# pylat/adaptive-proximal-algorithms

Hardware: NVIDIA B200
Metric: AdaPGM iters/sec on 65536x131072 fp64 lasso (higher is better)
Workload: dtype f64

## Files before the change

adaptive-proximal-algorithms_b200/csrc/api.cu:

```cuda
#include <algorithm>
#include <cmath>
#include <cstdlib>
#include <cstring>
#include <numeric>
#include "context.hpp"
#include "ops.cuh"
#include "solver_pd.cuh"
#include "solver_pg.cuh"
#include "solver_mp.cuh"
#include "solver_fused.cuh"
#include "solver_resident.cuh"
#include "solver_gridres.cuh"
#include "comm.hpp"

using namespace adaprox;

static int64_t round_up(int64_t v, int64_t a) { return (v + a - 1) / a * a; }

static int ws_reset(adaprox_ctx* h, size_t need) {
  if (need > h->ws_bytes) {
    if (h->ws) cudaFree(h->ws);
    h->ws = nullptr; h->ws_bytes = 0;
    size_t want = need + (need >> 3) + (1u << 20);
    cudaError_t e = cudaMalloc(&h->ws, want);
// ... 578 lines not shown
  if (cooperative && !std::getenv("ADAPROX_FUSED_NONCOOP")) {
    attrs[1].id = cudaLaunchAttributeCooperative;
    attrs[1].val.cooperative = 1;
    cfg->numAttrs = 2;
  }
  return ADAPROX_OK;
}

struct FusedPlan {
  cudaLaunchConfig_t cfg;
  cudaLaunchAttribute attrs[2];
  int Q = 0;
  int G = 0;
  FusedArgs fa{};
};
static int fused_plan(adaprox_ctx* h, const void* kernel, const DProblem& P, bool cooperative, FusedPlan* pl) {
  pl->fa = FusedArgs{};
  pl->fa.C = fused_cluster_size(P);
  int rc = fused_config(h, kernel, pl->fa.C, cooperative, &pl->cfg, pl->attrs, &pl->Q);
  if (rc) return rc;
  pl->G = pl->fa.C * pl->Q;
  pl->fa.tagged = cooperative ? 1 : 0;
  pl->fa.hV = 0; pl->fa.hR = 16;
#if ADAPROX_FUSED_VARIANT == 1
  if (cooperative && pl->fa.C == kFMaxCluster) {
    int V = (h->sm_count - pl->G) / kFMaxCluster;
    if (P.F.m / std::max(pl->Q, 1) < 4096) V = 0;
    if (const char* e = std::getenv("ADAPROX_HELPERS")) V = std::min((h->sm_count - pl->G) / kFMaxCluster, std::max(0, std::atoi(e)));
    pl->fa.hV = h->resident_dev ? std::min(V, 4) : 0;
    pl->fa.hHold = (int)(1.7 * pl->Q) + 1;
    if (const char* e = std::getenv("ADAPROX_HELPER_HOLD")) pl->fa.hHold = std::max(0, std::atoi(e));
    pl->fa.resident = h->resident_dev;
    pl->fa.resident_seq = ++h->solve_seq;
    if (const char* e = std::getenv("ADAPROX_HELPER_ROWS")) pl->fa.hR = std::min(64, std::max(1, std::atoi(e)));
  }
#endif
  pl->fa.npadf = (int64_t)pl->fa.C * kFCols;
  const int kper = (P.F.m / std::max(pl->Q, 1) >= 4096) ? 8 : 4;
  int64_t pw = (P.F.m + (int64_t)pl->Q * kper - 1) / ((int64_t)pl->Q * kper);
  pw = pw < 16 ? 16 : pw;
  if (const char* e = std::getenv("ADAPROX_FUSED_CHUNK")) { const int v = std::atoi(e); if (v >= 1) pw = v; }
  pl->fa.chunk_rows = (int)pw;
  pl->fa.nchunks = (int)((P.F.m + pw - 1) / pw);
  return 0;
}
static size_t fused_ws_bytes(const FusedPlan& pl) {
  return ws_size_doubles((int64_t)pl.fa.nchunks * pl.fa.npadf) + ws_size_doubles(pl.fa.nchunks) + 5 * ws_size_doubles(1) + ws_size_doubles(12) +
         ws_size_doubles((int64_t)4 * 2 * 64 * kFMaxCluster * kFGWarps) +
         ws_size_doubles(4 * 256) + ws_size_doubles(5 * kFTraceRows);
}
static int fused_ws_alloc(adaprox_ctx* h, FusedPlan* pl) {
  FusedArgs& fa = pl->fa;
  fa.gpartf = ws_doubles(h, (int64_t)fa.nchunks * fa.npadf);
  fa.fpart = ws_doubles(h, fa.nchunks);
  fa.bar = reinterpret_cast<unsigned long long*>(ws_doubles(h, 1));
  fa.next = reinterpret_cast<unsigned long long*>(ws_doubles(h, 1));
  fa.err = reinterpret_cast<int*>(ws_doubles(h, 1));
  fa.go = reinterpret_cast<unsigned long long*>(ws_doubles(h, 1));
  fa.done = reinterpret_cast<unsigned long long*>(ws_doubles(h, 1));
// ... 250 lines not shown
        at[0].val.clusterDim.x = kRCluster; at[0].val.clusterDim.y = 1; at[0].val.clusterDim.z = 1;
        cfg.gridDim = dim3(kRCluster, 1, 1); cfg.blockDim = dim3(kRThreads, 1, 1); cfg.dynamicSmemBytes = rsmem; cfg.stream = h->stream;
        cfg.attrs = at; cfg.numAttrs = 1;
        void* rargs[] = {&P, &O, &W, &rarg};
        cudaError_t e = cudaLaunchKernelExC(&cfg, (const void*)k_adapgm_resident, rargs);
        if (e != cudaSuccess) return fail(h, ADAPROX_ERR_CUDA, std::string("resident cluster launch: ") + cudaGetErrorString(e));
        h->launches++;
        rc = ADAPROX_OK;
      } else if (gridres) {
        void* gargs[] = {&P, &O, &W, &garg};
        cudaError_t e = cudaLaunchCooperativeKernel(gridres_kernel(o->solver), dim3(h->sm_count), dim3(kGThreads), gargs, gsmem, h->stream);
        if (e == cudaSuccess) {
          h->launches++;
          rc = ADAPROX_OK;
        } else {
          cudaGetLastError();
          gridres = false;
          rc = coop_launch(h, k_primal_dual<false>, args, Gcoop);
        }
      } else if (fused) {
        cudaError_t e = cudaLaunchKernelExC(&fpl.cfg, (const void*)k_adapgm_fused, fargs);
        if (e != cudaSuccess) return fail(h, ADAPROX_ERR_CUDA, std::string("fused cluster launch: ") + cudaGetErrorString(e));
        h->launches++;
#if ADAPROX_FUSED_VARIANT == 1
        if (fa.hV > 0) {
          bool up = false;
          for (long spin = 0; spin < 20000000L; ++spin) {
            if (*(volatile unsigned long long*)h->resident_host == fa.resident_seq) { up = true; break; }
            if ((spin & 1023) == 1023 && cudaStreamQuery(h->stream) != cudaErrorNotReady) break;
          }
          if (up && cudaFuncSetAttribute((const void*)k_adapgm_helper, cudaFuncAttributeMaxDynamicSharedMemorySize, kFRingBytes) == cudaSuccess &&
              cudaStreamWaitEvent(h->stream2, h->ev_h, 0) == cudaSuccess) {
            k_adapgm_helper<<<fa.hV * kFMaxCluster, kFThreads, kFRingBytes, h->stream2>>>(P, W, fa);
            if (cudaGetLastError() == cudaSuccess) { h->launches++; helper_launched = true; }
          } else {
            cudaGetLastError();
          }
        }
#endif
        rc = ADAPROX_OK;
      } else {
        rc = coop_launch(h, k_primal_dual<false>, args, Gcoop);
      }
      break;
    case ADAPROX_S_LINESEARCH_PRIMAL_DUAL:
      rc = coop_launch(h, k_primal_dual<true>, args, Gcoop);
      break;
    case ADAPROX_S_BACKTRACKING_PROXGRAD:
    case ADAPROX_S_BACKTRACKING_NESTEROV:
    case ADAPROX_S_FIXED_NESTEROV:
    case ADAPROX_S_AGRAAL:
      rc = 1;
      if (gridres) {
        void* gargs[] = {&P, &O, &W, &garg};
        if (cudaLaunchCooperativeKernel(gridres_kernel(o->solver), dim3(h->sm_count), dim3(kGThreads), gargs, gsmem, h->stream) == cudaSuccess) {
          h->launches++;
          rc = ADAPROX_OK;
        } else {
          cudaGetLastError();
          gridres = false;
        }
      }
// ... 111 lines not shown
```

adaptive-proximal-algorithms_b200/csrc/solver_fused.cuh:

```cuda
#pragma once
#include "phases.cuh"
#include "p2p.cuh"

namespace adaprox {

constexpr int kFGroup = 256;
constexpr int kFGWarps = kFGroup / 32;
constexpr int kFThreads = 2 * kFGroup;
constexpr int kFWarps = kFThreads / 32;
constexpr int kFCols = 8192;
constexpr int kFH = kFCols / 2 / kFGroup;
constexpr int kFStages = 3;
constexpr int kFStageBytes = kFCols * 8;
constexpr int kFRingBytes = kFStages * kFStageBytes;
constexpr int kFMaxCluster = 16;
#ifndef ADAPROX_FUSED_VARIANT
#define ADAPROX_FUSED_VARIANT 1
#endif
#if ADAPROX_FUSED_VARIANT == 1
constexpr int kFDepth = 8;
constexpr int kFXWarps = kFGWarps;
constexpr int kFsumThread = kFGroup;
#else
constexpr int kFDepth = 4;
constexpr int kFXWarps = kFWarps;
constexpr int kFsumThread = 0;
constexpr int kFH2 = kFCols / 2 / kFThreads;
#endif
constexpr int kFTraceRows = 512;
#ifdef ADAPROX_FUSED_TRACE
#define FTRACE(cond, k, i) do { if ((cond) && tr != nullptr && (i) < kFTraceRows) tr[(k) * kFTraceRows + (i)] = (unsigned long long)clock64(); } while (0)
#else
#define FTRACE(cond, k, i) do { } while (0)
#endif

struct FusedArgs {
  double* gpartf;
  double* fpart;
  int64_t npadf;
  int C;
  int chunk_rows;
  int nchunks;
  unsigned long long* bar;
  unsigned long long bar_base;
  unsigned long long* next;
  unsigned long long next_base;
  int sweep_only;
  const double* sh_x;
  double* sh_gbuf;
  const int* sh_done;
  P2PArgs p2p;
  int tagged;
  int hV, hR;
  int hHold;
  unsigned long long* go;
  unsigned long long* done;
  unsigned long long* hsync;
  double* hxch;
  unsigned long long* resident;
  unsigned long long resident_seq;
  int* err;
  unsigned long long* lat;
  unsigned long long* trace;
};

__device__ __forceinline__ uint32_t cluster_ctarank() { uint32_t r; asm volatile("mov.u32 %0, %%cluster_ctarank;" : "=r"(r)); return r; }
__device__ __forceinline__ uint32_t cluster_id_x() { uint32_t r; asm volatile("mov.u32 %0, %%clusterid.x;" : "=r"(r)); return r; }
__device__ __forceinline__ uint32_t ncluster_id_x() { uint32_t r; asm volatile("mov.u32 %0, %%nclusterid.x;" : "=r"(r)); return r; }
__device__ __forceinline__ void cluster_arrive() { asm volatile("barrier.cluster.arrive.release.aligned;" ::: "memory"); }
__device__ __forceinline__ void cluster_wait() { asm volatile("barrier.cluster.wait.acquire.aligned;" ::: "memory"); }

constexpr uint32_t kOffFull = 0, kOffEmpty = 8 * kFStages, kOffCfull = 16 * kFStages, kOffChunk = 16 * kFStages + 8 * kFDepth, kOffCpart = 128;
constexpr uint32_t kPartStride = kFMaxCluster * kFXWarps * 8;
constexpr uint32_t kOffRs = kOffCpart + kFDepth * kPartStride;
constexpr int kCtlBytes = kOffRs + kFDepth * 8;
static_assert(kOffChunk + 8 <= kOffCpart, "control block layout");

struct FusedSmem {
  uint32_t ring, ctl;
  uint32_t count;
};

__device__ __forceinline__ void st_async_peer(uint32_t local_data_addr, uint32_t local_mbar_addr, uint32_t peer, double v) {
  uint32_t rdata, rbar;
  asm volatile("mapa.shared::cluster.u32 %0, %1, %2;" : "=r"(rdata) : "r"(local_data_addr), "r"(peer));
  asm volatile("mapa.shared::cluster.u32 %0, %1, %2;" : "=r"(rbar) : "r"(local_mbar_addr), "r"(peer));
  asm volatile("st.async.weak.shared::cluster.mbarrier::complete_tx::bytes.b64 [%0], %1, [%2];"
               ::"r"(rdata), "l"(__double_as_longlong(v)), "r"(rbar) : "memory");
}
__device__ __forceinline__ void mbar_wait_cluster(uint32_t addr, uint32_t parity) {
  uint32_t ok;
  do {
    asm volatile("{\n\t.reg .pred p;\n\tmbarrier.try_wait.parity.acquire.cluster.shared::cta.b64 p, [%1], %2;\n\tselp.u32 %0, 1, 0, p;\n\t}"
                 : "=r"(ok) : "r"(addr), "r"(parity) : "memory");
  } while (!ok);
}

#ifndef ADAPROX_FUSED_TRYWAIT
__device__ __forceinline__ void fmbar_wait(uint32_t addr, uint32_t parity) {
  uint32_t ok;
  for (;;) {
    asm volatile("{\n\t.reg .pred p;\n\tmbarrier.test_wait.parity.shared::cta.b64 p, [%1], %2;\n\tselp.u32 %0, 1, 0, p;\n\t}"
                 : "=r"(ok) : "r"(addr), "r"(parity) : "memory");
    if (ok) break;
#ifdef ADAPROX_FUSED_POLL_SLEEP_NS
    __nanosleep(ADAPROX_FUSED_POLL_SLEEP_NS);
#endif
  }
}
#else
__device__ __forceinline__ void fmbar_wait(uint32_t addr, uint32_t parity) { mbar_wait(addr, parity); }
#endif

#if ADAPROX_FUSED_VARIANT == 1
constexpr int kFBarThreads = kFGroup;
#else
constexpr int kFBarThreads = kFThreads;
#endif
__device__ __forceinline__ void group_bar(int id) { asm volatile("bar.sync %0, %1;" ::"r"(id), "n"(kFBarThreads) : "memory"); }
#ifndef ADAPROX_FUSED_ALLPOLL
#ifndef ADAPROX_FUSED_TRYWAIT_NS
#define ADAPROX_FUSED_TRYWAIT_NS 64
#endif
#if ADAPROX_FUSED_TRYWAIT_NS <= 0
__device__ __forceinline__ void fmbar_wait_hint(uint32_t addr, uint32_t parity) { fmbar_wait(addr, parity); }
#else
__device__ __forceinline__ void fmbar_wait_hint(uint32_t addr, uint32_t parity) {
  uint32_t ok;
  do {
    asm volatile("{\n\t.reg .pred p;\n\tmbarrier.try_wait.parity.shared::cta.b64 p, [%1], %2, %3;\n\tselp.u32 %0, 1, 0, p;\n\t}"
                 : "=r"(ok) : "r"(addr), "r"(parity), "r"((uint32_t)ADAPROX_FUSED_TRYWAIT_NS) : "memory");
  } while (!ok);
}
#endif
__device__ __forceinline__ void group_wait(bool poller, int id, uint32_t addr, uint32_t parity) {
#if ADAPROX_FUSED_TRYWAIT_NS > 0
  if (poller) fmbar_wait_hint(addr, parity);
#elif defined(ADAPROX_FUSED_POLL_LANE0)
  if (poller) { if ((threadIdx.x & 31) == 0) fmbar_wait(addr, parity); __syncwarp(); }
#else
  if (poller) fmbar_wait(addr, parity);
#endif
  group_bar(id);
}
#else
__device__ __forceinline__ void group_wait(bool, int, uint32_t addr, uint32_t parity) { fmbar_wait(addr, parity); }
#endif

__device__ __forceinline__ double2 lds2v(uint32_t addr) {
  double2 v;
  asm volatile("ld.volatile.shared.v2.f64 {%0, %1}, [%2];" : "=d"(v.x), "=d"(v.y) : "r"(addr));
  return v;
}

#ifndef ADAPROX_FUSED_KFB
#define ADAPROX_FUSED_KFB 4
#endif
constexpr int kFB = ADAPROX_FUSED_KFB;

#if ADAPROX_FUSED_VARIANT == 1
__device__ __noinline__ double fused_pass(const DMat& M, const double* bvec, const double* x, FusedSmem& fs, int C,
                                           int64_t r0, int nrows, double* gout_row, unsigned long long* tr = nullptr) {
  const uint32_t ring = fs.ring, ctl = fs.ctl, g0 = fs.count;
  (void)tr;
  const uint32_t rank = cluster_ctarank();
  const int lane = threadIdx.x & 31, warp = threadIdx.x >> 5;
  const int64_t col0 = (int64_t)rank * kFCols;
  double fsum = 0.0;

  if (warp < kFGWarps) {
    const int t = threadIdx.x;
    double2 xr[kFH];
    {
      const int64_t n = M.n;
#pragma unroll
      for (int k = 0; k < kFH; ++k) {
        const int64_t j = col0 + 2 * (k * kFGroup + t);
        xr[k].x = (j < n) ? ldcg(x + j) : 0.0;
        xr[k].y = (j + 1 < n) ? ldcg(x + j + 1) : 0.0;
      }
    }
    uint32_t slot = g0 % kFStages, ph = (g0 / kFStages) & 1u, d = g0 % kFDepth;
    const uint32_t tile0 = ring + t * 16;
    const uint32_t mypart = ctl + kOffCpart + (rank * kFGWarps + warp) * 8;
    const bool sender = lane < C;
    uint32_t rdata0 = 0, rbar0 = 0;
    if (sender) {
      asm volatile("mapa.shared::cluster.u32 %0, %1, %2;" : "=r"(rdata0) : "r"(mypart), "r"((uint32_t)lane));
      asm volatile("mapa.shared::cluster.u32 %0, %1, %2;" : "=r"(rbar0) : "r"(ctl + kOffCfull), "r"((uint32_t)lane));
    }
    for (int i = 0; i < nrows; ++i) {
      group_wait(warp == 0, 1, ctl + kOffFull + 8 * slot, ph);
      FTRACE(t == 0, 1, i);
      const uint32_t tile = tile0 + slot * kFStageBytes;
      double p0 = 0.0, p1 = 0.0, p2 = 0.0, p3 = 0.0;
      double2 av[kFB];
#pragma unroll
      for (int h = 0; h < kFH; h += kFB) {
#pragma unroll
#ifdef ADAPROX_EXP_NO_DOT_LDS
        for (int k = 0; k < kFB; ++k) av[k] = xr[(h + k + 1) % kFH];
#else
        for (int k = 0; k < kFB; ++k) av[k] = lds2v(tile + (h + k) * kFGroup * 16);
#endif
#pragma unroll
        for (int k = kFB - 2; k >= 0; k -= 2) {
          p2 = fma(av[k + 1].x, xr[h + k + 1].x, p2);
          p3 = fma(av[k + 1].y, xr[h + k + 1].y, p3);
          p0 = fma(av[k].x, xr[h + k].x, p0);
          p1 = fma(av[k].y, xr[h + k].y, p1);
        }
      }
      const double pw = warp_sum((p0 + p1) + (p2 + p3));
      if (sender)
        asm volatile("st.async.weak.shared::cluster.mbarrier::complete_tx::bytes.b64 [%0], %1, [%2];"
                     ::"r"(rdata0 + d * kPartStride), "l"(__double_as_longlong(pw)), "r"(rbar0 + 8 * d) : "memory");
      FTRACE(t == 0, 2, i);
      if (++slot == kFStages) { slot = 0; ph ^= 1u; }
      d = (d + 1) % kFDepth;
    }
  } else {
    const int t = threadIdx.x - kFGroup;
    const bool leader = (t == 0);
    const bool producer = (t == kFGroup - 32);
    const int nval = C * kFGWarps;
    const uint32_t xbytes = (uint32_t)nval * 8;
    uint32_t bytes;
    {
      int64_t width = M.ld - col0;
      width = width < 0 ? 0 : (width > kFCols ? kFCols : width);
      bytes = (uint32_t)(width * 8);
    }
    const int64_t ldb = M.ld * 8;
    const char* src = reinterpret_cast<const char*>(M.a + col0 + r0 * M.ld);
    double2 acc[kFH];
#pragma unroll
    for (int k = 0; k < kFH; ++k) acc[k] = make_double2(0.0, 0.0);
    if (leader)
      for (int i = 0; i < kFDepth && i < nrows; ++i) mbar_expect_tx(ctl + kOffCfull + 8 * ((g0 + i) % kFDepth), xbytes);
    uint32_t slot = g0 % kFStages, ph = (g0 / kFStages) & 1u, d = g0 % kFDepth, dph = (g0 / kFDepth) & 1u;
    int issued = 0; (void)issued;
    const uint64_t pol = l2_policy_evict_first();
    auto issue = [&](uint32_t sl, uint32_t par) {
      fmbar_wait(ctl + kOffEmpty + 8 * sl, par ^ 1u);
      FTRACE(true, 0, issued); ++issued;
      mbar_expect_tx(ctl + kOffFull + 8 * sl, bytes);
      bulk_g2s_hint(ring + sl * kFStageBytes, src, bytes, ctl + kOffFull + 8 * sl, pol);
      src += ldb;
    };
    if (producer) {
      uint32_t sl = slot, par = ph;
      for (int i = 0; i < kFStages && i < nrows; ++i) {
        issue(sl, par);
        if (++sl == kFStages) { sl = 0; par ^= 1u; }
      }
    }
    const uint32_t tile0 = ring + t * 16;
    const uint32_t part0 = ctl + kOffCpart + lane * 8;
    const double* bp = bvec + r0;
    double bblk = 0.0;
    for (int i = 0; i < nrows; ++i) {
#if !defined(ADAPROX_FUSED_ALLPOLL) && !defined(ADAPROX_FUSED_ALL_REDUCE)
      if (warp == kFGWarps) {
        if ((i & 31) == 0) bblk = (i + lane < nrows) ? __ldg(bp + i + lane) : 0.0;
        const double b_cur = __shfl_sync(0xffffffffu, bblk, i & 31);
        fmbar_wait_hint(ctl + kOffCfull + 8 * d, dph);
        const uint32_t pb = part0 + d * kPartStride;
        const double v0 = (lane < nval) ? lds1(pb) : 0.0;
        const double v1 = (lane + 32 < nval) ? lds1(pb + 256) : 0.0;
        const double v2 = (lane + 64 < nval) ? lds1(pb + 512) : 0.0;
        const double v3 = (lane + 96 < nval) ? lds1(pb + 768) : 0.0;
        if (leader && i + kFDepth < nrows) mbar_expect_tx(ctl + kOffCfull + 8 * d, xbytes);
        const double r1 = warp_sum((v0 + v1) + (v2 + v3)) - b_cur;
        if (lane == 0) sts1(ctl + kOffRs + 8 * d, r1);
      }
      group_bar(2);
      FTRACE(leader, 3, i);
      const double rs = lds1(ctl + kOffRs + 8 * d);
#else
      if ((i & 31) == 0) bblk = (i + lane < nrows) ? __ldg(bp + i + lane) : 0.0;
      const double b_cur = __shfl_sync(0xffffffffu, bblk, i & 31);
      group_wait(warp == kFGWarps, 2, ctl + kOffCfull + 8 * d, dph);
      FTRACE(leader, 3, i);
      const uint32_t pb = part0 + d * kPartStride;
      const double v0 = (lane < nval) ? lds1(pb) : 0.0;
      const double v1 = (lane + 32 < nval) ? lds1(pb + 256) : 0.0;
      const double v2 = (lane + 64 < nval) ? lds1(pb + 512) : 0.0;
      const double v3 = (lane + 96 < nval) ? lds1(pb + 768) : 0.0;
      if (leader && i + kFDepth < nrows) mbar_expect_tx(ctl + kOffCfull + 8 * d, xbytes);
      const double rs = warp_sum((v0 + v1) + (v2 + v3)) - b_cur;
#endif
#ifdef ADAPROX_FUSED_ALLPOLL
      fmbar_wait(ctl + kOffFull + 8 * slot, ph);
#endif
      const uint32_t tile = tile0 + slot * kFStageBytes;
      double2 av[kFB];
#pragma unroll
      for (int h = 0; h < kFH; h += kFB) {
#pragma unroll
#ifdef ADAPROX_EXP_NO_UPD_LDS
        for (int k = 0; k < kFB; ++k) av[k] = make_double2(b_cur, rs);
#else
        for (int k = 0; k < kFB; ++k) av[k] = lds2v(tile + (h + k) * kFGroup * 16);
#endif
#ifndef ADAPROX_EXP_NO_SYNCWARP
        __syncwarp();
#endif
#pragma unroll
        for (int k = kFB - 1; k >= 0; --k) {
          acc[h + k].x = fma(av[k].x, rs, acc[h + k].x);
          acc[h + k].y = fma(av[k].y, rs, acc[h + k].y);
        }
      }
      __syncwarp();
      if (lane == 0) mbar_arrive(ctl + kOffEmpty + 8 * slot);
      FTRACE(leader, 4, i);
      if (producer && i + kFStages < nrows) issue(slot, ph ^ 1u);
      if (warp == kFGWarps) fsum = fma(rs, rs, fsum);
      if (++slot == kFStages) { slot = 0; ph ^= 1u; }
      if (++d == kFDepth) { d = 0; dph ^= 1u; }
    }
    double* gout = gout_row + col0;
#pragma unroll
    for (int k = 0; k < kFH; ++k) *reinterpret_cast<double2*>(gout + 2 * (k * kFGroup + t)) = acc[k];
    if (!(leader && rank == 0)) fsum = 0.0;
  }
  __syncthreads();
  fs.count = (uint32_t)(((uint64_t)g0 + (uint64_t)nrows) % 48u);
  return fsum;
}
#else
__device__ __noinline__ double fused_pass(const DMat& M, const double* bvec, const double* x, FusedSmem& fs, int C,
                                           int64_t r0, int nrows, double* gout_row, unsigned long long* tr = nullptr) {
  const uint32_t ring = fs.ring, ctl = fs.ctl, g0 = fs.count;
  (void)tr;
  const uint32_t rank = cluster_ctarank();
  const int t = threadIdx.x, lane = t & 31, warp = t >> 5;
  const int64_t col0 = (int64_t)rank * kFCols;
  double fsum = 0.0;

  double2 xr[kFH2], acc[kFH2];
  {
    const int64_t n = M.n;
#pragma unroll
    for (int k = 0; k < kFH2; ++k) {
      const int64_t j = col0 + 2 * (k * kFThreads + t);
      xr[k].x = (j < n) ? ldcg(x + j) : 0.0;
      xr[k].y = (j + 1 < n) ? ldcg(x + j + 1) : 0.0;
      acc[k] = make_double2(0.0, 0.0);
    }
  }
  const int nval = C * kFXWarps;
  const uint32_t xbytes = (uint32_t)nval * 8;
  uint32_t bytes;
  {
    int64_t width = M.ld - col0;
    width = width < 0 ? 0 : (width > kFCols ? kFCols : width);
    bytes = (uint32_t)(width * 8);
  }
  const int64_t ldb = M.ld * 8;
  const char* src = reinterpret_cast<const char*>(M.a + col0 + r0 * M.ld);
  uint32_t slot = g0 % kFStages, ph = (g0 / kFStages) & 1u, d = g0 % kFDepth, dph = (g0 / kFDepth) & 1u;
  auto issue = [&](uint32_t sl, uint32_t par) {
    fmbar_wait(ctl + kOffEmpty + 8 * sl, par ^ 1u);
    mbar_expect_tx(ctl + kOffFull + 8 * sl, bytes);
    bulk_g2s(ring + sl * kFStageBytes, src, bytes, ctl + kOffFull + 8 * sl);
    src += ldb;
  };
  if (t == 0) {
    for (int i = 0; i < kFDepth && i < nrows; ++i) mbar_expect_tx(ctl + kOffCfull + 8 * ((g0 + i) % kFDepth), xbytes);
    uint32_t sl = slot, par = ph;
    for (int i = 0; i < kFStages && i < nrows; ++i) {
      FTRACE(true, 0, i);
      issue(sl, par);
      if (++sl == kFStages) { sl = 0; par ^= 1u; }
    }
  }
  const uint32_t tile0 = ring + t * 16;
  const uint32_t mypart = ctl + kOffCpart + (rank * kFXWarps + warp) * 8;
  const uint32_t part0 = ctl + kOffCpart + lane * 8;
  const bool sender = lane < C;
  const double* bp = bvec + r0;
  double bblk = 0.0;
  for (int i = 0; i < nrows; ++i) {
    if ((i & 31) == 0) bblk = (i + lane < nrows) ? __ldg(bp + i + lane) : 0.0;
    const double b_cur = __shfl_sync(0xffffffffu, bblk, i & 31);
    group_wait(warp == 0, 1, ctl + kOffFull + 8 * slot, ph);
    FTRACE(t == 0, 1, i);
    const uint32_t tile = tile0 + slot * kFStageBytes;
    double2 av[kFH2];
#pragma unroll
    for (int k = 0; k < kFH2; ++k) av[k] = lds2v(tile + k * kFThreads * 16);
    double p0 = 0.0, p1 = 0.0, p2 = 0.0, p3 = 0.0;
#pragma unroll
    for (int k = kFH2 - 2; k >= 0; k -= 2) {
      p2 = fma(av[k + 1].x, xr[k + 1].x, p2);
      p3 = fma(av[k + 1].y, xr[k + 1].y, p3);
      p0 = fma(av[k].x, xr[k].x, p0);
      p1 = fma(av[k].y, xr[k].y, p1);
    }
    const double pw = warp_sum((p0 + p1) + (p2 + p3));
    if (lane == 0) mbar_arrive(ctl + kOffEmpty + 8 * slot);
    if (sender) st_async_peer(mypart + d * kPartStride, ctl + kOffCfull + 8 * d, (uint32_t)lane, pw);
    FTRACE(t == 0, 2, i);
    if (t == 0 && i + kFStages < nrows) { FTRACE(true, 0, i + kFStages); issue(slot, ph ^ 1u); }
    group_wait(warp == 1, 2, ctl + kOffCfull + 8 * d, dph);
    FTRACE(t == 0, 3, i);
    const uint32_t pb = part0 + d * kPartStride;
    double v[8];
#pragma unroll
    for (int k = 0; k < 8; ++k) v[k] = lds1(pb + 256 * k);
    const double rs = warp_sum(((v[0] + v[1]) + (v[2] + v[3])) + ((v[4] + v[5]) + (v[6] + v[7]))) - b_cur;
    __syncwarp();
    if (t == 0 && i + kFDepth < nrows) mbar_expect_tx(ctl + kOffCfull + 8 * d, xbytes);
#pragma unroll
    for (int k = 0; k < kFH2; ++k) {
      acc[k].x = fma(av[k].x, rs, acc[k].x);
      acc[k].y = fma(av[k].y, rs, acc[k].y);
    }
    FTRACE(t == 0, 4, i);
    fsum = fma(rs, rs, fsum);
    if (++slot == kFStages) { slot = 0; ph ^= 1u; }
    if (++d == kFDepth) { d = 0; dph ^= 1u; }
  }
  double* gout = gout_row + col0;
#pragma unroll
  for (int k = 0; k < kFH2; ++k) *reinterpret_cast<double2*>(gout + 2 * (k * kFThreads + t)) = acc[k];
  if (!(t == kFsumThread && rank == 0)) fsum = 0.0;
  __syncthreads();
  fs.count = (uint32_t)(((uint64_t)g0 + (uint64_t)nrows) % 24u);
  return fsum;
}
#endif

__device__ __forceinline__ void fused_sweep(const DMat& M, const double* bvec, const double* x, FusedSmem& fs, const FusedArgs& fa,
                                            unsigned long long sweep) {
  const uint32_t rank = cluster_ctarank();
  const unsigned long long base = fa.next_base + sweep * (unsigned long long)(fa.nchunks + (int)ncluster_id_x());
  const uint32_t mailbox = fs.ctl + kOffChunk;
  int taken = 0;
  for (;;) {
    if (rank == 0 && threadIdx.x == 0) {
      long long c;
      if (fa.tagged) {
        c = (long long)(atomicAdd(fa.next, 1ull) & 0xffffffffull);
      } else {
        c = (long long)(atomicAdd(fa.next, 1ull) - base);
      }
      for (int p = 0; p < fa.C; ++p) {
        uint32_t raddr;
        asm volatile("mapa.shared::cluster.u32 %0, %1, %2;" : "=r"(raddr) : "r"(mailbox), "r"(p));
        asm volatile("st.shared::cluster.s64 [%0], %1;" ::"r"(raddr), "l"(c) : "memory");
      }
    }
    cluster_arrive();
    cluster_wait();
    if (fa.tagged && taken > 0 && rank == 0 && threadIdx.x == 0) { __threadfence(); atomicAdd(fa.done, 1ull); }
    long long c;
    asm volatile("ld.volatile.shared.s64 %0, [%1];" : "=l"(c) : "r"(mailbox));
    if (c >= fa.nchunks) break;
    const int64_t r0 = c * (int64_t)fa.chunk_rows;
    const int64_t left = M.m - r0;
    const int nrows = (int)(left < fa.chunk_rows ? left : fa.chunk_rows);
#ifdef ADAPROX_FUSED_TRACE
    const double fv = fused_pass(M, bvec, x, fs, fa.C, r0, nrows, fa.gpartf + c * fa.npadf, (blockIdx.x == 0 && taken == 1) ? fa.trace : nullptr);
#else
    const double fv = fused_pass(M, bvec, x, fs, fa.C, r0, nrows, fa.gpartf + c * fa.npadf);
#endif
    if (rank == 0 && threadIdx.x == kFsumThread) fa.fpart[c] = fv;
    ++taken;
  }
  if (fa.lat && threadIdx.x == 0) fa.lat[4 * blockIdx.x] += (unsigned long long)taken;
}

__device__ __forceinline__ void fused_gradient_slice(const FusedArgs& fa, int64_t j0, int64_t j1, double* out) {
  for (int64_t j = j0 + threadIdx.x; j < j1; j += kFThreads) {
    const double* p = fa.gpartf + j;
    double s = 0.0;
    int c = 0;
    for (; c + 8 <= fa.nchunks; c += 8) {
      double v[8];
#pragma unroll
      for (int k = 0; k < 8; ++k) v[k] = ldcg(p + (int64_t)(c + k) * fa.npadf);
#pragma unroll
      for (int k = 0; k < 8; ++k) s += v[k];
    }
    for (; c < fa.nchunks; ++c) s += ldcg(p + (int64_t)c * fa.npadf);
    out[j] = s;
  }
}
__device__ __forceinline__ double fused_fsum(const FusedArgs& fa, uint32_t scr) {
  const int lane = threadIdx.x & 31;
// ... 50 lines not shown
      __threadfence();
      atomicAdd(ctr, 1ull);
      unsigned long long seen, t0 = 0;
      for (unsigned spin = 0;; ++spin) {
        asm volatile("ld.acquire.gpu.global.u64 %0, [%1];" : "=l"(seen) : "l"(ctr) : "memory");
        if (seen >= target) break;
        if ((spin & 4095u) == 4095u) {
          if (*reinterpret_cast<volatile int*>(err)) break;
          const unsigned long long now = globaltimer_ns();
          if (t0 == 0) t0 = now;
          else if (now - t0 > kGridBarTimeoutNs) { *reinterpret_cast<volatile int*>(err) = 1; __threadfence(); break; }
        }
      }
    }
    __syncthreads();
  }
};

__device__ __forceinline__ void fused_smem_init(FusedSmem& fs, unsigned char* dyn_smem, unsigned char* s_ctl, int64_t ld) {
  fs.ring = smem_u32(dyn_smem);
  fs.ctl = smem_u32(s_ctl);
  fs.count = 0;
  if (threadIdx.x == 0) {
    for (int s = 0; s < kFStages; ++s) { mbar_init(fs.ctl + kOffFull + 8 * s, 1); mbar_init(fs.ctl + kOffEmpty + 8 * s, kFXWarps); }
    for (int s = 0; s < kFDepth; ++s) mbar_init(fs.ctl + kOffCfull + 8 * s, 1);
    asm volatile("fence.mbarrier_init.release.cluster;" ::: "memory");
  }
  {
    int64_t width = ld - (int64_t)cluster_ctarank() * kFCols;
    width = width < 0 ? 0 : (width > kFCols ? kFCols : width);
    for (int s = 0; s < kFStages; ++s)
      for (int64_t j = width + threadIdx.x; j < kFCols; j += kFThreads) sts1(fs.ring + s * kFStageBytes + (uint32_t)j * 8, 0.0);
  }
  for (int j = threadIdx.x; j < (int)(kFDepth * kPartStride / 8); j += kFThreads) sts1(fs.ctl + kOffCpart + j * 8, 0.0);
  __syncthreads();
  cluster_arrive();
  cluster_wait();
}

__global__ void __launch_bounds__(kFThreads, 1) k_adapgm_fused(DProblem P, DOpts O, DWork W, FusedArgs fa) {
  GridBar grid{fa.bar, 0ull, gridDim.x, fa.err};
  const int b = blockIdx.x, G = gridDim.x;
  extern __shared__ __align__(1024) unsigned char dyn_smem[];
  __shared__ __align__(16) unsigned char s_ctl[kCtlBytes];
  __shared__ double s_scr[kFWarps * 8 + kMaxRed];
  FusedSmem fs;
  fused_smem_init(fs, dyn_smem, s_ctl, P.F.ld);
  const uint32_t scr = smem_u32(s_scr);

  const bool want_obj = O.want_objective != 0;
  int64_t j0, j1;
  cta_slice(P.n, b, G, j0, j1);
  unsigned long long sweep = 0;

  if (fa.sweep_only) {
    grid.target = fa.bar_base;
    const bool done = __ldcg(fa.sh_done) != 0;
    if (!done) {
      unsigned long long tq0 = 0;
      if (fa.lat && threadIdx.x == 0) tq0 = globaltimer_ns();
// ... 1 lines not shown
      if (fa.lat && threadIdx.x == 0) { fa.lat[4 * b + 1] = globaltimer_ns() - tq0; unsigned sm; asm volatile("mov.u32 %0, %%smid;" : "=r"(sm)); fa.lat[4 * b + 3] = sm; }
    }
    grid.sync();
    if (fa.p2p.n <= 1) {
      if (!done) {
        fused_gradient_slice(fa, j0, j1, fa.sh_gbuf);
        const double f0 = fused_fsum(fa, scr);
        if (b == 0 && threadIdx.x == 0) { fa.sh_gbuf[P.n] = f0; fa.sh_gbuf[P.n + 1] = 0.0; }
      }
    } else {
      P2PState ps;
      p2p_begin(fa.p2p, ps);
      if (!done) {
        fused_gradient_slice(fa, j0, j1, fa.sh_gbuf);
        const double f0 = fused_fsum(fa, scr);
        if (b == 0 && threadIdx.x == 0) { fa.sh_gbuf[P.n] = f0; fa.sh_gbuf[P.n + 1] = 0.0; }
      }
      grid.sync();
      if (!done) p2p_allreduce<kFThreads>(fa.p2p, ps, grid, fa.sh_gbuf, fa.sh_gbuf, P.n + 2);
      else { grid.sync(); grid.sync(); }
    }
    cluster_arrive();
    cluster_wait();
    return;
  }

  double gamma, sigma, s0, s1;
  rule_init(O, gamma, sigma, s0, s1);
  int64_t n_eval = 0, n_grad = 0, n_proxg = 0, n_rec = 0;
  unsigned flags = 0;
  int xc = 0, gc = 0;
  double* x = W.xb[0];
  if (fa.hV > 0) {
    grid.sync();
    if (b == 0 && threadIdx.x == 0) asm volatile("st.release.sys.global.u64 [%0], %1;" ::"l"(fa.resident), "l"(fa.resident_seq) : "memory");
  }
  const bool sharded = fa.p2p.n > 1;
  P2PState ps;
  p2p_begin(fa.p2p, ps);
  auto arm_sweep = [&](unsigned long long s_next) {
    if (fa.tagged && b == 0 && threadIdx.x == 0) asm volatile("st.relaxed.gpu.global.u64 [%0], %1;" ::"l"(fa.next), "l"(s_next << 32) : "memory");
  };
  auto release_sweep = [&](unsigned long long s_next) {
    if (fa.tagged && fa.hV > 0 && b == 0 && threadIdx.x == 0) asm volatile("st.release.gpu.global.u64 [%0], %1;" ::"l"(fa.go), "l"(s_next) : "memory");
  };
  auto wait_chunks = [&](unsigned long long sweeps_done) {
// ... 128 lines not shown
    grid.sync();
    release_sweep(sweep);
    phase_stamp(W, it, 7);
  }
  if (fa.tagged && b == 0 && threadIdx.x == 0) {
    asm volatile("st.release.gpu.global.u64 [%0], %1;" ::"l"(fa.next), "l"(0xffffffffull << 32) : "memory");
    if (fa.hV > 0) asm volatile("st.release.gpu.global.u64 [%0], %1;" ::"l"(fa.go), "l"(~0ull) : "memory");
  }

  const int64_t tid = (int64_t)b * kFThreads + threadIdx.x, nt = (int64_t)G * kFThreads;
  for (int64_t j = tid; j < P.n; j += nt) W.xout[j] = x[j];
  if (b == 0 && threadIdx.x == 0) {
    DResult r;
    r.iters = it_done;
    r.flags = flags | (converged ? ADAPROX_FLAG_CONVERGED : 0u);
    r.xbuf = 0;
    r.f_evals = n_eval; r.grad_f_evals = n_grad; r.prox_g_evals = n_proxg; r.prox_h_evals = 0;
    r.A_evals = 0; r.At_evals = 0; r.n_records = n_rec;
    r.final_gamma = gamma; r.final_sigma = sigma; r.final_norm_res = norm_res;
    *W.res = r;
  }
  cluster_arrive();
  cluster_wait();
}

}

#include "solver_fused_helper.cuh"
```

adaptive-proximal-algorithms_b200/csrc/solver_fused_helper.cuh:

```cuda
#pragma once

namespace adaprox {

#if ADAPROX_FUSED_VARIANT == 1

constexpr unsigned long long kHelperRollCallNs = 50000000ull;
constexpr unsigned long long kHelperIdleNs = 60000000000ull;
constexpr unsigned long long kExitTag = 0xffffffffull;

struct VcBar {
  unsigned long long* ctr;
  unsigned long long target;
  int* err;
  __device__ __forceinline__ void sync() {
    __syncthreads();
    if (threadIdx.x == 0) {
      target += kFMaxCluster;
      __threadfence();
      atomicAdd(ctr, 1ull);
      unsigned long long seen, t0 = 0;
      for (unsigned spin = 0;; ++spin) {
        asm volatile("ld.acquire.gpu.global.u64 %0, [%1];" : "=l"(seen) : "l"(ctr) : "memory");
        if (seen >= target) break;
        if ((spin & 4095u) == 4095u) {
          if (*reinterpret_cast<volatile int*>(err)) break;
          const unsigned long long now = globaltimer_ns();
          if (t0 == 0) t0 = now;
// ... 224 lines not shown
          const uint32_t slot = gg % kFStages, ph = (gg / kFStages) & 1u;
          fmbar_wait_hint(empty0 + 8 * slot, ph ^ 1u);
          mbar_expect_tx(full0 + 8 * slot, bytes);
          bulk_g2s_hint(ring + slot * kFStageBytes, src, bytes, full0 + 8 * slot, pol);
          src += ldb;
          gg = (gg + 1) % 6u;
        }
      }
      g = (g + (uint32_t)nb) % 6u;
      ++batch_no;
      __syncthreads();
    }
    if (warp >= kFGWarps) {
      double* gout = gout_row + col0;
#pragma unroll
      for (int k = 0; k < kFH; ++k) *reinterpret_cast<double2*>(gout + 2 * (k * kFGroup + tg)) = acc[k];
      if (tg == 0 && rho == 0) fa.fpart[c] = fsum;
    }
    vb.sync();
    if (rho == 0 && t == 0) { __threadfence(); atomicAdd(fa.done, 1ull); atomicAdd(fa.hsync + 10, 1ull); }
  }
}

#endif

}
```

Before: 89.69.

## Stage matrix rows through tensor memory to free the smem ring early

Measured after the change: 95.46 (median of 6 runs). +6.4%, better.

```diff
diff --git a/adaptive-proximal-algorithms_b200/csrc/api.cu b/adaptive-proximal-algorithms_b200/csrc/api.cu
--- a/adaptive-proximal-algorithms_b200/csrc/api.cu
+++ b/adaptive-proximal-algorithms_b200/csrc/api.cu
@@ -624,7 +624,6 @@
   pl->G = pl->fa.C * pl->Q;
   pl->fa.tagged = cooperative ? 1 : 0;
   pl->fa.hV = 0; pl->fa.hR = 16;
-#if ADAPROX_FUSED_VARIANT == 1
   if (cooperative && pl->fa.C == kFMaxCluster) {
     int V = (h->sm_count - pl->G) / kFMaxCluster;
     if (P.F.m / std::max(pl->Q, 1) < 4096) V = 0;
@@ -636,7 +635,6 @@
     pl->fa.resident_seq = ++h->solve_seq;
     if (const char* e = std::getenv("ADAPROX_HELPER_ROWS")) pl->fa.hR = std::min(64, std::max(1, std::atoi(e)));
   }
-#endif
   pl->fa.npadf = (int64_t)pl->fa.C * kFCols;
   const int kper = (P.F.m / std::max(pl->Q, 1) >= 4096) ? 8 : 4;
   int64_t pw = (P.F.m + (int64_t)pl->Q * kper - 1) / ((int64_t)pl->Q * kper);
@@ -933,7 +931,6 @@
         cudaError_t e = cudaLaunchKernelExC(&fpl.cfg, (const void*)k_adapgm_fused, fargs);
         if (e != cudaSuccess) return fail(h, ADAPROX_ERR_CUDA, std::string("fused cluster launch: ") + cudaGetErrorString(e));
         h->launches++;
-#if ADAPROX_FUSED_VARIANT == 1
         if (fa.hV > 0) {
           bool up = false;
           for (long spin = 0; spin < 20000000L; ++spin) {
@@ -948,7 +945,6 @@
             cudaGetLastError();
           }
         }
-#endif
         rc = ADAPROX_OK;
       } else {
         rc = coop_launch(h, k_primal_dual<false>, args, Gcoop);
diff --git a/adaptive-proximal-algorithms_b200/csrc/solver_fused.cuh b/adaptive-proximal-algorithms_b200/csrc/solver_fused.cuh
--- a/adaptive-proximal-algorithms_b200/csrc/solver_fused.cuh
+++ b/adaptive-proximal-algorithms_b200/csrc/solver_fused.cuh
@@ -14,19 +14,11 @@
 constexpr int kFStageBytes = kFCols * 8;
 constexpr int kFRingBytes = kFStages * kFStageBytes;
 constexpr int kFMaxCluster = 16;
-#ifndef ADAPROX_FUSED_VARIANT
-#define ADAPROX_FUSED_VARIANT 1
-#endif
-#if ADAPROX_FUSED_VARIANT == 1
 constexpr int kFDepth = 8;
-constexpr int kFXWarps = kFGWarps;
-constexpr int kFsumThread = kFGroup;
-#else
-constexpr int kFDepth = 4;
-constexpr int kFXWarps = kFWarps;
-constexpr int kFsumThread = 0;
-constexpr int kFH2 = kFCols / 2 / kFThreads;
-#endif
+constexpr int kFTBufs = 4;
+constexpr int kFTCols = 512;
+constexpr int kFTBufCols = kFTCols / kFTBufs;
+static_assert(kFTBufCols == 2 * kFH * 4, "a buffer holds a row of the two dot warps of a lane quarter: 2 x 16 double2 per lane");
 constexpr int kFTraceRows = 512;
 #ifdef ADAPROX_FUSED_TRACE
 #define FTRACE(cond, k, i) do { if ((cond) && tr != nullptr && (i) < kFTraceRows) tr[(k) * kFTraceRows + (i)] = (unsigned long long)clock64(); } while (0)
@@ -71,15 +63,41 @@
 __device__ __forceinline__ void cluster_wait() { asm volatile("barrier.cluster.wait.acquire.aligned;" ::: "memory"); }
 
 constexpr uint32_t kOffFull = 0, kOffEmpty = 8 * kFStages, kOffCfull = 16 * kFStages, kOffChunk = 16 * kFStages + 8 * kFDepth, kOffCpart = 128;
-constexpr uint32_t kPartStride = kFMaxCluster * kFXWarps * 8;
+constexpr uint32_t kPartStride = kFMaxCluster * kFGWarps * 8;
 constexpr uint32_t kOffRs = kOffCpart + kFDepth * kPartStride;
-constexpr int kCtlBytes = kOffRs + kFDepth * 8;
+constexpr uint32_t kOffTempty = kOffRs + kFDepth * 8;
+constexpr uint32_t kOffTmem = kOffTempty + kFTBufs * 8;
+constexpr int kCtlBytes = kOffTmem + 8;
 static_assert(kOffChunk + 8 <= kOffCpart, "control block layout");
 
 struct FusedSmem {
   uint32_t ring, ctl;
+  uint32_t tmem;
   uint32_t count;
 };
+
+__device__ __forceinline__ void tmem_st_batch(uint32_t taddr, const double2 (&v)[4]) {
+  asm volatile("tcgen05.st.sync.aligned.32x32b.x16.b32 [%0], {%1, %2, %3, %4, %5, %6, %7, %8, %9, %10, %11, %12, %13, %14, %15, %16};"
+               ::"r"(taddr),
+                 "r"(__double2loint(v[0].x)), "r"(__double2hiint(v[0].x)), "r"(__double2loint(v[0].y)), "r"(__double2hiint(v[0].y)),
+                 "r"(__double2loint(v[1].x)), "r"(__double2hiint(v[1].x)), "r"(__double2loint(v[1].y)), "r"(__double2hiint(v[1].y)),
+                 "r"(__double2loint(v[2].x)), "r"(__double2hiint(v[2].x)), "r"(__double2loint(v[2].y)), "r"(__double2hiint(v[2].y)),
+                 "r"(__double2loint(v[3].x)), "r"(__double2hiint(v[3].x)), "r"(__double2loint(v[3].y)), "r"(__double2hiint(v[3].y))
+               : "memory");
+}
+__device__ __forceinline__ void tmem_ld_batch(uint32_t taddr, double2 (&v)[4]) {
+  int w[16];
+  asm volatile("tcgen05.ld.sync.aligned.32x32b.x16.b32 {%0, %1, %2, %3, %4, %5, %6, %7, %8, %9, %10, %11, %12, %13, %14, %15}, [%16];\n\t"
+               "tcgen05.wait::ld.sync.aligned;"
+               : "=r"(w[0]), "=r"(w[1]), "=r"(w[2]), "=r"(w[3]), "=r"(w[4]), "=r"(w[5]), "=r"(w[6]), "=r"(w[7]),
+                 "=r"(w[8]), "=r"(w[9]), "=r"(w[10]), "=r"(w[11]), "=r"(w[12]), "=r"(w[13]), "=r"(w[14]), "=r"(w[15])
+               : "r"(taddr) : "memory");
+#pragma unroll
+  for (int k = 0; k < 4; ++k) v[k] = make_double2(__hiloint2double(w[4 * k + 1], w[4 * k]), __hiloint2double(w[4 * k + 3], w[4 * k + 2]));
+}
+__device__ __forceinline__ void tmem_wait_st() { asm volatile("tcgen05.wait::st.sync.aligned;" ::: "memory"); }
+__device__ __forceinline__ void tmem_fence_before_sync() { asm volatile("tcgen05.fence::before_thread_sync;" ::: "memory"); }
+__device__ __forceinline__ void tmem_fence_after_sync() { asm volatile("tcgen05.fence::after_thread_sync;" ::: "memory"); }
 
 __device__ __forceinline__ void st_async_peer(uint32_t local_data_addr, uint32_t local_mbar_addr, uint32_t peer, double v) {
   uint32_t rdata, rbar;
@@ -112,12 +130,7 @@
 __device__ __forceinline__ void fmbar_wait(uint32_t addr, uint32_t parity) { mbar_wait(addr, parity); }
 #endif
 
-#if ADAPROX_FUSED_VARIANT == 1
-constexpr int kFBarThreads = kFGroup;
-#else
-constexpr int kFBarThreads = kFThreads;
-#endif
-__device__ __forceinline__ void group_bar(int id) { asm volatile("bar.sync %0, %1;" ::"r"(id), "n"(kFBarThreads) : "memory"); }
+__device__ __forceinline__ void group_bar(int id) { asm volatile("bar.sync %0, %1;" ::"r"(id), "n"(kFGroup) : "memory"); }
 #ifndef ADAPROX_FUSED_ALLPOLL
 #ifndef ADAPROX_FUSED_TRYWAIT_NS
 #define ADAPROX_FUSED_TRYWAIT_NS 64
@@ -133,18 +146,30 @@
   } while (!ok);
 }
 #endif
+__device__ __forceinline__ void poller_wait(uint32_t addr, uint32_t parity) {
+#if ADAPROX_FUSED_TRYWAIT_NS > 0
+  fmbar_wait_hint(addr, parity);
+#elif defined(ADAPROX_FUSED_POLL_LANE0)
+  if ((threadIdx.x & 31) == 0) fmbar_wait(addr, parity);
+  __syncwarp();
+#else
+  fmbar_wait(addr, parity);
+#endif
+}
 __device__ __forceinline__ void group_wait(bool poller, int id, uint32_t addr, uint32_t parity) {
-#if ADAPROX_FUSED_TRYWAIT_NS > 0
-  if (poller) fmbar_wait_hint(addr, parity);
-#elif defined(ADAPROX_FUSED_POLL_LANE0)
-  if (poller) { if ((threadIdx.x & 31) == 0) fmbar_wait(addr, parity); __syncwarp(); }
-#else
-  if (poller) fmbar_wait(addr, parity);
-#endif
+  if (poller) poller_wait(addr, parity);
+  group_bar(id);
+}
+__device__ __forceinline__ void group_wait(bool poller, int id, uint32_t addr, uint32_t parity, uint32_t addr2, uint32_t parity2) {
+  if (poller) { poller_wait(addr, parity); poller_wait(addr2, parity2); }
   group_bar(id);
 }
 #else
 __device__ __forceinline__ void group_wait(bool, int, uint32_t addr, uint32_t parity) { fmbar_wait(addr, parity); }
+__device__ __forceinline__ void group_wait(bool, int, uint32_t addr, uint32_t parity, uint32_t addr2, uint32_t parity2) {
+  fmbar_wait(addr, parity);
+  fmbar_wait(addr2, parity2);
+}
 #endif
 
 __device__ __forceinline__ double2 lds2v(uint32_t addr) {
@@ -153,23 +178,45 @@
   return v;
 }
 
-#ifndef ADAPROX_FUSED_KFB
-#define ADAPROX_FUSED_KFB 4
-#endif
-constexpr int kFB = ADAPROX_FUSED_KFB;
-
-#if ADAPROX_FUSED_VARIANT == 1
-__device__ __noinline__ double fused_pass(const DMat& M, const double* bvec, const double* x, FusedSmem& fs, int C,
-                                           int64_t r0, int nrows, double* gout_row, unsigned long long* tr = nullptr) {
+constexpr int kFB = 4;
+
+__device__ __noinline__ void fused_pass(const DMat& M, const double* bvec, const double* x, FusedSmem& fs, int C,
+                                         int64_t r0, int nrows, double* gout_row, double* fout, unsigned long long* tr = nullptr) {
   const uint32_t ring = fs.ring, ctl = fs.ctl, g0 = fs.count;
+  fs.count = (uint32_t)(((uint64_t)g0 + (uint64_t)nrows) % 48u);
   (void)tr;
   const uint32_t rank = cluster_ctarank();
   const int lane = threadIdx.x & 31, warp = threadIdx.x >> 5;
   const int64_t col0 = (int64_t)rank * kFCols;
-  double fsum = 0.0;
+  const uint32_t tq = fs.tmem + ((uint32_t)(warp & 3) << 21) + (uint32_t)((warp >> 2) & 1) * (kFTBufCols / 2);
 
   if (warp < kFGWarps) {
     const int t = threadIdx.x;
+    const bool producer = (t == kFGroup - 32);
+    uint32_t slot = g0 % kFStages, ph = (g0 / kFStages) & 1u, d = g0 % kFDepth, tb = g0 % kFTBufs, tph = (g0 / kFTBufs) & 1u;
+    uint32_t bytes;
+    {
+      int64_t width = M.ld - col0;
+      width = width < 0 ? 0 : (width > kFCols ? kFCols : width);
+      bytes = (uint32_t)(width * 8);
+    }
+    const uint32_t ldb = (uint32_t)(M.ld * 8);
+    const char* src = reinterpret_cast<const char*>(M.a + col0 + r0 * M.ld);
+    int issued = 0; (void)issued;
+    auto issue = [&](uint32_t sl, uint32_t par) {
+      fmbar_wait(ctl + kOffEmpty + 8 * sl, par ^ 1u);
+      FTRACE(true, 0, issued); ++issued;
+      mbar_expect_tx(ctl + kOffFull + 8 * sl, bytes);
+      bulk_g2s_hint(ring + sl * kFStageBytes, src, bytes, ctl + kOffFull + 8 * sl, l2_policy_evict_first());
+      src += ldb;
+    };
+    if (producer) {
+      uint32_t sl = slot, par = ph;
+      for (int i = 0; i < kFStages && i < nrows; ++i) {
+        issue(sl, par);
+        if (++sl == kFStages) { sl = 0; par ^= 1u; }
+      }
+    }
     double2 xr[kFH];
     {
       const int64_t n = M.n;
@@ -180,7 +227,6 @@
         xr[k].y = (j + 1 < n) ? ldcg(x + j + 1) : 0.0;
       }
     }
-    uint32_t slot = g0 % kFStages, ph = (g0 / kFStages) & 1u, d = g0 % kFDepth;
     const uint32_t tile0 = ring + t * 16;
     const uint32_t mypart = ctl + kOffCpart + (rank * kFGWarps + warp) * 8;
     const bool sender = lane < C;
@@ -190,9 +236,11 @@
       asm volatile("mapa.shared::cluster.u32 %0, %1, %2;" : "=r"(rbar0) : "r"(ctl + kOffCfull), "r"((uint32_t)lane));
     }
     for (int i = 0; i < nrows; ++i) {
-      group_wait(warp == 0, 1, ctl + kOffFull + 8 * slot, ph);
+      group_wait(warp == 0, 1, ctl + kOffTempty + 8 * tb, tph ^ 1u, ctl + kOffFull + 8 * slot, ph);
+      tmem_fence_after_sync();
       FTRACE(t == 0, 1, i);
       const uint32_t tile = tile0 + slot * kFStageBytes;
+      const uint32_t trow = tq + tb * kFTBufCols;
       double p0 = 0.0, p1 = 0.0, p2 = 0.0, p3 = 0.0;
       double2 av[kFB];
 #pragma unroll
@@ -210,52 +258,34 @@
           p0 = fma(av[k].x, xr[h + k].x, p0);
           p1 = fma(av[k].y, xr[h + k].y, p1);
         }
-      }
+        tmem_st_batch(trow + 4 * h, av);
+      }
+      __syncwarp();
+      if (lane == 0) mbar_arrive(ctl + kOffEmpty + 8 * slot);
+      FTRACE(t == 0, 2, i);
       const double pw = warp_sum((p0 + p1) + (p2 + p3));
+      tmem_wait_st();
+      tmem_fence_before_sync();
       if (sender)
         asm volatile("st.async.weak.shared::cluster.mbarrier::complete_tx::bytes.b64 [%0], %1, [%2];"
                      ::"r"(rdata0 + d * kPartStride), "l"(__double_as_longlong(pw)), "r"(rbar0 + 8 * d) : "memory");
-      FTRACE(t == 0, 2, i);
+      if (producer && i + kFStages < nrows) issue(slot, ph ^ 1u);
       if (++slot == kFStages) { slot = 0; ph ^= 1u; }
       d = (d + 1) % kFDepth;
+      if (++tb == kFTBufs) { tb = 0; tph ^= 1u; }
     }
   } else {
     const int t = threadIdx.x - kFGroup;
     const bool leader = (t == 0);
-    const bool producer = (t == kFGroup - 32);
     const int nval = C * kFGWarps;
     const uint32_t xbytes = (uint32_t)nval * 8;
-    uint32_t bytes;
-    {
-      int64_t width = M.ld - col0;
-      width = width < 0 ? 0 : (width > kFCols ? kFCols : width);
-      bytes = (uint32_t)(width * 8);
-    }
-    const int64_t ldb = M.ld * 8;
-    const char* src = reinterpret_cast<const char*>(M.a + col0 + r0 * M.ld);
     double2 acc[kFH];
 #pragma unroll
     for (int k = 0; k < kFH; ++k) acc[k] = make_double2(0.0, 0.0);
     if (leader)
       for (int i = 0; i < kFDepth && i < nrows; ++i) mbar_expect_tx(ctl + kOffCfull + 8 * ((g0 + i) % kFDepth), xbytes);
-    uint32_t slot = g0 % kFStages, ph = (g0 / kFStages) & 1u, d = g0 % kFDepth, dph = (g0 / kFDepth) & 1u;
-    int issued = 0; (void)issued;
-    const uint64_t pol = l2_policy_evict_first();
-    auto issue = [&](uint32_t sl, uint32_t par) {
-      fmbar_wait(ctl + kOffEmpty + 8 * sl, par ^ 1u);
-      FTRACE(true, 0, issued); ++issued;
-      mbar_expect_tx(ctl + kOffFull + 8 * sl, bytes);
-      bulk_g2s_hint(ring + sl * kFStageBytes, src, bytes, ctl + kOffFull + 8 * sl, pol);
-      src += ldb;
-    };
-    if (producer) {
-      uint32_t sl = slot, par = ph;
-      for (int i = 0; i < kFStages && i < nrows; ++i) {
-        issue(sl, par);
-        if (++sl == kFStages) { sl = 0; par ^= 1u; }
-      }
-    }
-    const uint32_t tile0 = ring + t * 16;
+    uint32_t d = g0 % kFDepth, dph = (g0 / kFDepth) & 1u, tb = g0 % kFTBufs;
+    double fsum = 0.0;
     const uint32_t part0 = ctl + kOffCpart + lane * 8;
     const double* bp = bvec + r0;
     double bblk = 0.0;
@@ -290,148 +320,33 @@
       if (leader && i + kFDepth < nrows) mbar_expect_tx(ctl + kOffCfull + 8 * d, xbytes);
       const double rs = warp_sum((v0 + v1) + (v2 + v3)) - b_cur;
 #endif
-#ifdef ADAPROX_FUSED_ALLPOLL
-      fmbar_wait(ctl + kOffFull + 8 * slot, ph);
-#endif
-      const uint32_t tile = tile0 + slot * kFStageBytes;
+      tmem_fence_after_sync();
+      const uint32_t trow = tq + tb * kFTBufCols;
       double2 av[kFB];
 #pragma unroll
       for (int h = 0; h < kFH; h += kFB) {
-#pragma unroll
-#ifdef ADAPROX_EXP_NO_UPD_LDS
-        for (int k = 0; k < kFB; ++k) av[k] = make_double2(b_cur, rs);
-#else
-        for (int k = 0; k < kFB; ++k) av[k] = lds2v(tile + (h + k) * kFGroup * 16);
-#endif
-#ifndef ADAPROX_EXP_NO_SYNCWARP
-        __syncwarp();
-#endif
+        tmem_ld_batch(trow + 4 * h, av);
 #pragma unroll
         for (int k = kFB - 1; k >= 0; --k) {
           acc[h + k].x = fma(av[k].x, rs, acc[h + k].x);
           acc[h + k].y = fma(av[k].y, rs, acc[h + k].y);
         }
       }
+      tmem_fence_before_sync();
       __syncwarp();
-      if (lane == 0) mbar_arrive(ctl + kOffEmpty + 8 * slot);
+      if (lane == 0) mbar_arrive(ctl + kOffTempty + 8 * tb);
       FTRACE(leader, 4, i);
-      if (producer && i + kFStages < nrows) issue(slot, ph ^ 1u);
       if (warp == kFGWarps) fsum = fma(rs, rs, fsum);
-      if (++slot == kFStages) { slot = 0; ph ^= 1u; }
       if (++d == kFDepth) { d = 0; dph ^= 1u; }
+      if (++tb == kFTBufs) tb = 0;
     }
     double* gout = gout_row + col0;
 #pragma unroll
     for (int k = 0; k < kFH; ++k) *reinterpret_cast<double2*>(gout + 2 * (k * kFGroup + t)) = acc[k];
-    if (!(leader && rank == 0)) fsum = 0.0;
+    if (leader && rank == 0) *fout = fsum;
   }
   __syncthreads();
-  fs.count = (uint32_t)(((uint64_t)g0 + (uint64_t)nrows) % 48u);
-  return fsum;
-}
-#else
-__device__ __noinline__ double fused_pass(const DMat& M, const double* bvec, const double* x, FusedSmem& fs, int C,
-                                           int64_t r0, int nrows, double* gout_row, unsigned long long* tr = nullptr) {
-  const uint32_t ring = fs.ring, ctl = fs.ctl, g0 = fs.count;
-  (void)tr;
-  const uint32_t rank = cluster_ctarank();
-  const int t = threadIdx.x, lane = t & 31, warp = t >> 5;
-  const int64_t col0 = (int64_t)rank * kFCols;
-  double fsum = 0.0;
-
-  double2 xr[kFH2], acc[kFH2];
-  {
-    const int64_t n = M.n;
-#pragma unroll
-    for (int k = 0; k < kFH2; ++k) {
-      const int64_t j = col0 + 2 * (k * kFThreads + t);
-      xr[k].x = (j < n) ? ldcg(x + j) : 0.0;
-      xr[k].y = (j + 1 < n) ? ldcg(x + j + 1) : 0.0;
-      acc[k] = make_double2(0.0, 0.0);
-    }
-  }
-  const int nval = C * kFXWarps;
-  const uint32_t xbytes = (uint32_t)nval * 8;
-  uint32_t bytes;
-  {
-    int64_t width = M.ld - col0;
-    width = width < 0 ? 0 : (width > kFCols ? kFCols : width);
-    bytes = (uint32_t)(width * 8);
-  }
-  const int64_t ldb = M.ld * 8;
-  const char* src = reinterpret_cast<const char*>(M.a + col0 + r0 * M.ld);
-  uint32_t slot = g0 % kFStages, ph = (g0 / kFStages) & 1u, d = g0 % kFDepth, dph = (g0 / kFDepth) & 1u;
-  auto issue = [&](uint32_t sl, uint32_t par) {
-    fmbar_wait(ctl + kOffEmpty + 8 * sl, par ^ 1u);
-    mbar_expect_tx(ctl + kOffFull + 8 * sl, bytes);
-    bulk_g2s(ring + sl * kFStageBytes, src, bytes, ctl + kOffFull + 8 * sl);
-    src += ldb;
-  };
-  if (t == 0) {
-    for (int i = 0; i < kFDepth && i < nrows; ++i) mbar_expect_tx(ctl + kOffCfull + 8 * ((g0 + i) % kFDepth), xbytes);
-    uint32_t sl = slot, par = ph;
-    for (int i = 0; i < kFStages && i < nrows; ++i) {
-      FTRACE(true, 0, i);
-      issue(sl, par);
-      if (++sl == kFStages) { sl = 0; par ^= 1u; }
-    }
-  }
-  const uint32_t tile0 = ring + t * 16;
-  const uint32_t mypart = ctl + kOffCpart + (rank * kFXWarps + warp) * 8;
-  const uint32_t part0 = ctl + kOffCpart + lane * 8;
-  const bool sender = lane < C;
-  const double* bp = bvec + r0;
-  double bblk = 0.0;
-  for (int i = 0; i < nrows; ++i) {
-    if ((i & 31) == 0) bblk = (i + lane < nrows) ? __ldg(bp + i + lane) : 0.0;
-    const double b_cur = __shfl_sync(0xffffffffu, bblk, i & 31);
-    group_wait(warp == 0, 1, ctl + kOffFull + 8 * slot, ph);
-    FTRACE(t == 0, 1, i);
-    const uint32_t tile = tile0 + slot * kFStageBytes;
-    double2 av[kFH2];
-#pragma unroll
-    for (int k = 0; k < kFH2; ++k) av[k] = lds2v(tile + k * kFThreads * 16);
-    double p0 = 0.0, p1 = 0.0, p2 = 0.0, p3 = 0.0;
-#pragma unroll
-    for (int k = kFH2 - 2; k >= 0; k -= 2) {
-      p2 = fma(av[k + 1].x, xr[k + 1].x, p2);
-      p3 = fma(av[k + 1].y, xr[k + 1].y, p3);
-      p0 = fma(av[k].x, xr[k].x, p0);
-      p1 = fma(av[k].y, xr[k].y, p1);
-    }
-    const double pw = warp_sum((p0 + p1) + (p2 + p3));
-    if (lane == 0) mbar_arrive(ctl + kOffEmpty + 8 * slot);
-    if (sender) st_async_peer(mypart + d * kPartStride, ctl + kOffCfull + 8 * d, (uint32_t)lane, pw);
-    FTRACE(t == 0, 2, i);
-    if (t == 0 && i + kFStages < nrows) { FTRACE(true, 0, i + kFStages); issue(slot, ph ^ 1u); }
-    group_wait(warp == 1, 2, ctl + kOffCfull + 8 * d, dph);
-    FTRACE(t == 0, 3, i);
-    const uint32_t pb = part0 + d * kPartStride;
-    double v[8];
-#pragma unroll
-    for (int k = 0; k < 8; ++k) v[k] = lds1(pb + 256 * k);
-    const double rs = warp_sum(((v[0] + v[1]) + (v[2] + v[3])) + ((v[4] + v[5]) + (v[6] + v[7]))) - b_cur;
-    __syncwarp();
-    if (t == 0 && i + kFDepth < nrows) mbar_expect_tx(ctl + kOffCfull + 8 * d, xbytes);
-#pragma unroll
-    for (int k = 0; k < kFH2; ++k) {
-      acc[k].x = fma(av[k].x, rs, acc[k].x);
-      acc[k].y = fma(av[k].y, rs, acc[k].y);
-    }
-    FTRACE(t == 0, 4, i);
-    fsum = fma(rs, rs, fsum);
-    if (++slot == kFStages) { slot = 0; ph ^= 1u; }
-    if (++d == kFDepth) { d = 0; dph ^= 1u; }
-  }
-  double* gout = gout_row + col0;
-#pragma unroll
-  for (int k = 0; k < kFH2; ++k) *reinterpret_cast<double2*>(gout + 2 * (k * kFThreads + t)) = acc[k];
-  if (!(t == kFsumThread && rank == 0)) fsum = 0.0;
-  __syncthreads();
-  fs.count = (uint32_t)(((uint64_t)g0 + (uint64_t)nrows) % 24u);
-  return fsum;
-}
-#endif
+}
 
 __device__ __forceinline__ void fused_sweep(const DMat& M, const double* bvec, const double* x, FusedSmem& fs, const FusedArgs& fa,
                                             unsigned long long sweep) {
@@ -463,11 +378,10 @@
     const int64_t left = M.m - r0;
     const int nrows = (int)(left < fa.chunk_rows ? left : fa.chunk_rows);
 #ifdef ADAPROX_FUSED_TRACE
-    const double fv = fused_pass(M, bvec, x, fs, fa.C, r0, nrows, fa.gpartf + c * fa.npadf, (blockIdx.x == 0 && taken == 1) ? fa.trace : nullptr);
+    fused_pass(M, bvec, x, fs, fa.C, r0, nrows, fa.gpartf + c * fa.npadf, fa.fpart + c, (blockIdx.x == 0 && taken == 1) ? fa.trace : nullptr);
 #else
-    const double fv = fused_pass(M, bvec, x, fs, fa.C, r0, nrows, fa.gpartf + c * fa.npadf);
-#endif
-    if (rank == 0 && threadIdx.x == kFsumThread) fa.fpart[c] = fv;
+    fused_pass(M, bvec, x, fs, fa.C, r0, nrows, fa.gpartf + c * fa.npadf, fa.fpart + c);
+#endif
     ++taken;
   }
   if (fa.lat && threadIdx.x == 0) fa.lat[4 * blockIdx.x] += (unsigned long long)taken;
@@ -564,8 +478,9 @@
   fs.ctl = smem_u32(s_ctl);
   fs.count = 0;
   if (threadIdx.x == 0) {
-    for (int s = 0; s < kFStages; ++s) { mbar_init(fs.ctl + kOffFull + 8 * s, 1); mbar_init(fs.ctl + kOffEmpty + 8 * s, kFXWarps); }
+    for (int s = 0; s < kFStages; ++s) { mbar_init(fs.ctl + kOffFull + 8 * s, 1); mbar_init(fs.ctl + kOffEmpty + 8 * s, kFGWarps); }
     for (int s = 0; s < kFDepth; ++s) mbar_init(fs.ctl + kOffCfull + 8 * s, 1);
+    for (int s = 0; s < kFTBufs; ++s) mbar_init(fs.ctl + kOffTempty + 8 * s, kFGWarps);
     asm volatile("fence.mbarrier_init.release.cluster;" ::: "memory");
   }
   {
@@ -575,9 +490,22 @@
       for (int64_t j = width + threadIdx.x; j < kFCols; j += kFThreads) sts1(fs.ring + s * kFStageBytes + (uint32_t)j * 8, 0.0);
   }
   for (int j = threadIdx.x; j < (int)(kFDepth * kPartStride / 8); j += kFThreads) sts1(fs.ctl + kOffCpart + j * 8, 0.0);
+  if (threadIdx.x < 32) {
+    asm volatile("tcgen05.alloc.cta_group::1.sync.aligned.shared::cta.b32 [%0], %1;" ::"r"(fs.ctl + kOffTmem), "n"(kFTCols) : "memory");
+    asm volatile("tcgen05.relinquish_alloc_permit.cta_group::1.sync.aligned;" ::: "memory");
+  }
+  tmem_fence_before_sync();
   __syncthreads();
+  tmem_fence_after_sync();
+  asm volatile("ld.shared.u32 %0, [%1];" : "=r"(fs.tmem) : "r"(fs.ctl + kOffTmem) : "memory");
   cluster_arrive();
   cluster_wait();
+}
+__device__ __forceinline__ void fused_tmem_free(const FusedSmem& fs) {
+  if (threadIdx.x < 32) {
+    tmem_fence_after_sync();
+    asm volatile("tcgen05.dealloc.cta_group::1.sync.aligned.b32 %0, %1;" ::"r"(fs.tmem), "n"(kFTCols) : "memory");
+  }
 }
 
 __global__ void __launch_bounds__(kFThreads, 1) k_adapgm_fused(DProblem P, DOpts O, DWork W, FusedArgs fa) {
@@ -625,6 +553,7 @@
     }
     cluster_arrive();
     cluster_wait();
+    fused_tmem_free(fs);
     return;
   }
 
@@ -799,6 +728,7 @@
   }
   cluster_arrive();
   cluster_wait();
+  fused_tmem_free(fs);
 }
 
 }
diff --git a/adaptive-proximal-algorithms_b200/csrc/solver_fused_helper.cuh b/adaptive-proximal-algorithms_b200/csrc/solver_fused_helper.cuh
--- a/adaptive-proximal-algorithms_b200/csrc/solver_fused_helper.cuh
+++ b/adaptive-proximal-algorithms_b200/csrc/solver_fused_helper.cuh
@@ -1,8 +1,6 @@
 #pragma once
 
 namespace adaprox {
-
-#if ADAPROX_FUSED_VARIANT == 1
 
 constexpr unsigned long long kHelperRollCallNs = 50000000ull;
 constexpr unsigned long long kHelperIdleNs = 60000000000ull;
@@ -273,6 +271,4 @@
   }
 }
 
-#endif
-
 }
```
